# xyvirtualgroup/AdaptivePnP_SCI

Measured on NVIDIA B200. Metric: admm_iters_per_sec, higher is better.
Workload: dtype f16 operands / f32 accumulate (inference convs); tf32 / f32 (online update); f32 elsewhere

## Files before the change

adaptivepnp_sci_b200/csrc/sci_conv_tc.cu:

```cuda
#include <cuda.h>
#include <cuda_fp16.h>
#include <stdlib.h>

#include "sci_common.cuh"

int sci_conv3x3_ref_launch(const sci_conv_desc* d, void* stream);
int sci_wgrad_ref_launch(const sci_wgrad_desc* d, void* stream);

namespace {

constexpr int TILE_W = 16, TILE_H = 8;
constexpr int KCH = 32;
constexpr int A_BYTES = TILE_W * TILE_H * KCH * 4;
constexpr int TC_THREADS = 256;
constexpr int MAX_STAGES = 8;

struct FwdParams {
    const float* scale; const float* shift; const float* residual; float* y;
    int N, H, W, Ho, Wo, Cin, Cout, stride, relu, ps, round_tf32, wsplit, emit_lo;
    int tiles_w, tiles_h, num_tiles, k_chunks, stages, acc_stride, tmem_cols;
    int Cstore;
    int ks_last;
    int rb_in, a_bytes;
    int lo_chunk0;
// ... 282 lines not shown
                        for (int j = 0; j < 32; j += 8) {
                            uint32_t h[4];
#pragma unroll
                            for (int e = 0; e < 4; ++e) {
                                float t0 = v[j + 2 * e] * s_scale[c0 + j + 2 * e] + s_shift[c0 + j + 2 * e];
                                float t1 = v[j + 2 * e + 1] * s_scale[c0 + j + 2 * e + 1] + s_shift[c0 + j + 2 * e + 1];
                                if (p.relu) { t0 = fmaxf(t0, 0.f); t1 = fmaxf(t1, 0.f); }
                                h[e] = pack_half2(t0, t1);
                            }
                            if (j < nc) *reinterpret_cast<uint4*>(yp + j) = make_uint4(h[0], h[1], h[2], h[3]);
                        }
                    }
                } else if (valid) {
                    long o;
                    if (p.ps) {
                        const int qq = c0 / Cq, cc = c0 % Cq;
                        o = (((long)n * 2 * p.Ho + 2 * ho + (qq >> 1)) * 2 * p.Wo + 2 * wo + (qq & 1)) * Cq + cc;
                    } else {
                        o = (((long)n * p.Ho + ho) * p.Wo + wo) * (p.Cout << p.emit_lo) + c0;
                    }
#pragma unroll
                    for (int j = 0; j < 32; j += 4) {
                        if (j >= nc) break;
                        float4 r4 = make_float4(0.f, 0.f, 0.f, 0.f);
                        if (p.residual) r4 = *reinterpret_cast<const float4*>(p.residual + o + j);
                        float out[4], lo[4];
                        const float rr[4] = {r4.x, r4.y, r4.z, r4.w};
#pragma unroll
                        for (int e = 0; e < 4; ++e) {
                            float t = v[j + e] * s_scale[c0 + j + e] + s_shift[c0 + j + e];
                            if (p.relu) t = fmaxf(t, 0.f);
                            t += rr[e];
                            const float hi = p.round_tf32 ? rna_tf32(t) : t;
                            lo[e] = rna_tf32(t - hi);
                            out[e] = hi;
                        }
                        *reinterpret_cast<float4*>(p.y + o + j) = make_float4(out[0], out[1], out[2], out[3]);
                        if (p.emit_lo)
                            *reinterpret_cast<float4*>(p.y + o + p.Cout + j) = make_float4(lo[0], lo[1], lo[2], lo[3]);
                    }
                }
            }
            tc_fence_before();
            __syncwarp();
            if (lane == 0) mbar_arrive(&tempty_bar[acc]);
            if (++acc == 2) { acc = 0; acc_phase ^= 1u; }
        }
        if (lane == 0) asm volatile("cp.async.bulk.wait_group 0;" ::: "memory");
    }
    tc_fence_before();
    __syncthreads();
    if (warp == 2) {
        tc_fence_after();
        asm volatile("tcgen05.dealloc.cta_group::1.sync.aligned.b32 %0, %1;" ::"r"(tmem_base), "r"((uint32_t)p.tmem_cols) : "memory");
    }
}


constexpr int ROW_PX = 130;
constexpr int ROW_BYTES = ROW_PX * KCH * 4;
constexpr int A2_STAGE = 17 * 1024;

struct Fwd2Params {
    const float* scale; const float* shift; const float* residual; float* y;
    int N, H, W, Cin, Cout, relu, ps, round_tf32;
    int tiles_w, num_tiles, k_chunks, stages, acc_stride, tmem_cols, resident, out_bufs;
    const float* planar_in1; float* planar_out;
    int pdl;
    int col0, Ctot;
    int stack;
    int R, tiles_h;
    int dbg;
    int ucols, Cstore;
    const float* mask_y; float* col_s1; float* col_s2; int mask_relu;
    int split;
    int ks_last;
    int rb_in, rb_out, a_stage, row_bytes;
    uint32_t desc_hi;
};

template <int EPI_WG, int MODE, bool HALF>
__global__ void __launch_bounds__(128 + 128 * EPI_WG, 1)
conv_fwd2_tc_kernel(const __grid_constant__ CUtensorMap tmA, const __grid_constant__ CUtensorMap tmB,
                    const __grid_constant__ CUtensorMap tmY, const Fwd2Params p) {
    extern __shared__ uint8_t smem_raw[];
    __shared__ __align__(8) uint64_t full_bar[MAX_STAGES], empty_bar[MAX_STAGES], tfull_bar[2], tempty_bar[2], w_bar;
    __shared__ uint32_t tmem_slot;
    __shared__ __align__(16) float s_scale[128], s_shift[128];
    __shared__ float s_cs1[MODE == 4 ? 128 : 1], s_cs2[MODE == 4 ? 128 : 1];

    const int warp = threadIdx.x >> 5, lane = threadIdx.x & 31;
    if (MODE == 4) {
        for (int i = threadIdx.x; i < 128; i += 128 + 128 * EPI_WG) { s_cs1[i] = 0.f; s_cs2[i] = 0.f; }
    }
    const uint32_t smem_base = (smem_u32(smem_raw) + 1023u) & ~1023u;
    const uint32_t b_bytes = (uint32_t)p.Cout * (uint32_t)p.rb_in;
    const uint32_t w_bytes = p.resident ? 9u * (uint32_t)p.k_chunks * b_bytes : 0u;
    const bool wpair = !p.resident && p.R == 2;
    const uint32_t stage_bytes = (uint32_t)p.a_stage * (wpair ? 2u : 1u) + (p.resident ? 0u : 3u * b_bytes);
    const uint32_t ring_base = smem_base + w_bytes;
    const uint32_t stage_out_base = ring_base + (uint32_t)p.stages * stage_bytes;

    for (int i = threadIdx.x; i < p.Cout; i += 128 + 128 * EPI_WG) {
        s_scale[i] = p.scale ? p.scale[p.col0 + i] : 1.f;
        s_shift[i] = p.shift ? p.shift[p.col0 + i] : 0.f;
    }
    if (warp == 0 && lane == 0) {
        asm volatile("prefetch.tensormap [%0];" ::"l"(&tmA) : "memory");
        asm volatile("prefetch.tensormap [%0];" ::"l"(&tmB) : "memory");
    }
    if (warp == 1 && lane == 0) {
        for (int s = 0; s < p.stages; ++s) { mbar_init(&full_bar[s], 1); mbar_init(&empty_bar[s], 1); }
        for (int a = 0; a < 2; ++a) { mbar_init(&tfull_bar[a], 1); mbar_init(&tempty_bar[a], 4 * EPI_WG); }
        mbar_init(&w_bar, 1);
        asm volatile("fence.mbarrier_init.release.cluster;" ::: "memory");
        asm volatile("fence.proxy.async.shared::cta;" ::: "memory");
    }
    if (warp == 2) {
        asm volatile("tcgen05.alloc.cta_group::1.sync.aligned.shared::cta.b32 [%0], %1;" ::"r"(smem_u32(&tmem_slot)), "r"((uint32_t)p.tmem_cols) : "memory");
        asm volatile("tcgen05.relinquish_alloc_permit.cta_group::1.sync.aligned;" ::: "memory");
    }
    tc_fence_before();
    __syncthreads();
    tc_fence_after();
    const uint32_t tmem_base = __shfl_sync(0xffffffffu, tmem_slot, 0);
    asm volatile("griddepcontrol.launch_dependents;" ::: "memory");

    if (warp == 0) {
        if (p.resident) {
            if (elect_one()) {
                mbar_arrive_expect_tx(&w_bar, w_bytes);
                for (int tap = 0; tap < 9; ++tap)
                    for (int kc = 0; kc < p.k_chunks; ++kc) {
                        const uint32_t slot = p.stack ? (uint32_t)(((tap % 3) * p.k_chunks + kc) * 3 + tap / 3)
                                                      : (uint32_t)(tap * p.k_chunks + kc);
                        tma_load_3d(smem_base + slot * b_bytes, &tmB, &w_bar, kc * (HALF ? (p.rb_in >> 1) : KCH), p.col0, tap);
                    }
            }
            __syncwarp();
        }
        if (p.pdl) asm volatile("griddepcontrol.wait;" ::: "memory");
        int stage = 0; uint32_t phase = 0;
        for (int tile = blockIdx.x; tile < p.num_tiles; tile += gridDim.x) {
            const int wt = tile % p.tiles_w, hg = (tile / p.tiles_w) % p.tiles_h, n = tile / (p.tiles_w * p.tiles_h);
            const int y0 = hg * p.R, rows = min(p.R, p.H - y0);
            if (wpair) {
                for (int r = 0; r < 3; ++r) {
                    for (int kc = 0; kc < p.k_chunks; ++kc) {
                        mbar_wait(&empty_bar[stage], phase ^ 1u);
                        if (elect_one()) {
                            mbar_arrive_expect_tx(&full_bar[stage], 2u * (uint32_t)p.row_bytes + 3u * b_bytes);
                            const uint32_t a_dst = ring_base + (uint32_t)stage * stage_bytes;
                            const int cc = kc * (HALF ? (p.rb_in >> 1) : KCH);
                            tma_load_4d(a_dst, &tmA, &full_bar[stage], cc, wt * 128 - 1, y0 + r - 1, n);
                            tma_load_4d(a_dst + (uint32_t)p.a_stage, &tmA, &full_bar[stage], cc, wt * 128 - 1, y0 + r, n);
                            for (int s = 0; s < 3; ++s)
                                tma_load_3d(a_dst + 2u * (uint32_t)p.a_stage + (uint32_t)s * b_bytes, &tmB, &full_bar[stage], cc, p.col0, r * 3 + s);
                        }
                        __syncwarp();
                        if (++stage == p.stages) { stage = 0; phase ^= 1u; }
                    }
                }
                continue;
            }
            for (int j = 0; j < rows + 2; ++j) {
                for (int kc = 0; kc < p.k_chunks; ++kc) {
                    mbar_wait(&empty_bar[stage], phase ^ 1u);
                    if (elect_one()) {
                        const bool skip_a = (p.dbg & 2) != 0;
                        mbar_arrive_expect_tx(&full_bar[stage], (skip_a ? 0u : (uint32_t)p.row_bytes) + (p.resident ? 0u : 3u * b_bytes));
                        const uint32_t a_dst = ring_base + (uint32_t)stage * stage_bytes;
                        if (!skip_a) tma_load_4d(a_dst, &tmA, &full_bar[stage], kc * (HALF ? (p.rb_in >> 1) : KCH), wt * 128 - 1, y0 + j - 1, n);
                        if (!p.resident) {
                            for (int s = 0; s < 3; ++s)
                                tma_load_3d(a_dst + (uint32_t)p.a_stage + (uint32_t)s * b_bytes, &tmB, &full_bar[stage], kc * (HALF ? (p.rb_in >> 1) : KCH), p.col0, j * 3 + s);
                        }
                    }
                    __syncwarp();
                    if (++stage == p.stages) { stage = 0; phase ^= 1u; }
                }
            }
        }
    } else if (warp == 1) {
        const bool leader = elect_one();
        const uint32_t idesc = mma_idesc(HALF, p.Cout);
        if (p.resident) { mbar_wait(&w_bar, 0); tc_fence_after(); }
        int stage = 0; uint32_t phase = 0; int acc = 0; uint32_t acc_phase = 0;
        const uint32_t b_tile_lo = b_bytes >> 4;
        const uint32_t tapu = (uint32_t)p.rb_in >> 4;
        const int ks_full = p.rb_in >> 5;
        for (int tile = blockIdx.x; tile < p.num_tiles; tile += gridDim.x) {
            mbar_wait(&tempty_bar[acc], acc_phase ^ 1u);
            tc_fence_after();
            const int hg = (tile / p.tiles_w) % p.tiles_h;
            const int rows = min(p.R, p.H - hg * p.R);
            const uint32_t d_base = tmem_base + (uint32_t)(acc * p.R * p.acc_stride);
            if (p.R == 1) {
// ... 70 lines not shown
                    const int nr = r_hi - r_lo + 1;
                    const uint32_t d_col = d_base + (uint32_t)((p.R - 1 - (j - r_lo)) * p.acc_stride);
                    const uint32_t idesc_n = (idesc & ~(0x3Fu << 17)) | ((uint32_t)((nr * p.Cout) >> 3) << 17);
                    const uint32_t idesc_m = (idesc & ~(0x3Fu << 17)) | ((uint32_t)(((nr - 1) * p.Cout) >> 3) << 17);
                    for (int kc = 0; kc < p.k_chunks; ++kc) {
                        mbar_wait(&full_bar[stage], phase);
                        tc_fence_after();
                        if (leader) {
                            const uint32_t a_lo = desc_lo(ring_base + (uint32_t)stage * stage_bytes);
                            const int ksn = (kc == p.k_chunks - 1) ? p.ks_last : ks_full;
                            const uint32_t b_lo = desc_lo(smem_base + (uint32_t)(kc * 3 + r_lo) * b_bytes);
                            const uint32_t b_step = (uint32_t)(3 * p.k_chunks) * b_tile_lo;
                            if (p.dbg & 1) {
                            } else if (r_lo == 0 && kc == 0) {
                                mma_lo<HALF>(d_col, a_lo, b_lo, idesc, 0u, p.desc_hi);
                                if (nr > 1) mma_lo<HALF>(d_col + (uint32_t)p.acc_stride, a_lo, b_lo + b_tile_lo, idesc_m, 1u, p.desc_hi);
#pragma unroll
                                for (int sk = 1; sk < 3 * (KCH / 8); ++sk) {
                                    const int s = sk / (KCH / 8), k = sk % (KCH / 8);
                                    if (k < ksn) mma_lo<HALF>(d_col, a_lo + s * tapu + k * 2, b_lo + s * b_step + k * 2, idesc_n, 1u, p.desc_hi);
                                }
                            } else {
#pragma unroll
                                for (int s = 0; s < 3; ++s) {
#pragma unroll
                                    for (int k = 0; k < KCH / 8; ++k)
                                        if (k < ksn) mma_lo<HALF>(d_col, a_lo + s * tapu + k * 2, b_lo + s * b_step + k * 2, idesc_n, 1u, p.desc_hi);
                                }
                            }
                            tc_commit(&empty_bar[stage]);
                        }
                        __syncwarp();
                        if (++stage == p.stages) { stage = 0; phase ^= 1u; }
                    }
                }
            } else {
                for (int j = 0; j < rows + 2; ++j) {
                    for (int kc = 0; kc < p.k_chunks; ++kc) {
                        mbar_wait(&full_bar[stage], phase);
                        tc_fence_after();
                        if (leader) {
                            const uint32_t a_addr = ring_base + (uint32_t)stage * stage_bytes;
                            const uint32_t a_lo = desc_lo(a_addr);
                            const int ksn = (kc == p.k_chunks - 1) ? p.ks_last : ks_full;
                            for (int t = max(0, j - 2); t <= min(rows - 1, j); ++t) {
                                const int r = j - t;
                                const uint32_t d_tmem = d_base + (uint32_t)(t * p.acc_stride);
                                const uint32_t b_lo = desc_lo(p.resident ? smem_base + (uint32_t)(r * 3 * p.k_chunks + kc) * b_bytes : a_addr + (uint32_t)p.a_stage);
                                const uint32_t b_step = p.resident ? (uint32_t)p.k_chunks * b_tile_lo : b_tile_lo;
                                const uint32_t first = (uint32_t)((r | kc) != 0);
                                if (!(p.dbg & 1)) {
#pragma unroll
                                    for (int s = 0; s < 3; ++s) {
#pragma unroll
                                        for (int k = 0; k < KCH / 8; ++k)
                                            if (k < ksn) mma_lo<HALF>(d_tmem, a_lo + s * tapu + k * 2, b_lo + s * b_step + k * 2, idesc, (s | k) ? 1u : first, p.desc_hi);
                                    }
                                }
                            }
                            tc_commit(&empty_bar[stage]);
                        }
                        __syncwarp();
                        if (++stage == p.stages) { stage = 0; phase ^= 1u; }
                    }
                }
            }
            if (leader) tc_commit(&tfull_bar[acc]);
            __syncwarp();
            if (++acc == 2) { acc = 0; acc_phase ^= 1u; }
        }
    } else if (warp >= 4) {
        const int q = warp & 3;
        const int g = (warp >> 2) - 1;
        const int m = q * 32 + lane;
        const int Cq = p.Ctot >> 2;
        const int nch = p.Cout >> 5;
        const float lower = p.relu ? 0.f : -INFINITY;
        const long pl_plane = (long)p.H * p.W;
        constexpr int PIN_ROWS = (8 + EPI_WG - 1) / EPI_WG;
        const uint32_t tile_b = (uint32_t)p.rb_out * 32u;
        const uint32_t sbuf0 = stage_out_base + (uint32_t)((g * 4 + q) * p.out_bufs) * tile_b;
        int acc = 0; uint32_t acc_phase = 0;
        uint32_t st_cnt = 0;
        if (p.pdl) asm volatile("griddepcontrol.wait;" ::: "memory");
        for (int tile = blockIdx.x; tile < p.num_tiles; tile += gridDim.x) {
            const int wt = tile % p.tiles_w, hg = (tile / p.tiles_w) % p.tiles_h, n = tile / (p.tiles_w * p.tiles_h);
            const int y0 = hg * p.R, rows = min(p.R, p.H - y0);
            const int wo = wt * 128 + m;
            const bool valid = wo < p.W;
            const int units = rows * nch;
            auto out_offset = [&](int ho, int c0) -> long {
                const int cg = p.col0 + c0;
                if (p.ps) {
                    const int qq = cg / Cq, cc = cg % Cq;
                    return (((long)n * 2 * p.H + 2 * ho + (qq >> 1)) * 2 * p.W + 2 * wo + (qq & 1)) * Cq + cc;
                }
                return (((long)n * p.H + ho) * p.W + wo) * p.Ctot + cg;
            };
            float4 rr[8];
            float pin[PIN_ROWS][3];
            if (!HALF && MODE == 1) {
#pragma unroll
                for (int j = 0; j < 8; ++j) rr[j] = make_float4(0.f, 0.f, 0.f, 0.f);
                if (p.residual && valid && g < units) {
                    const float4* rp = reinterpret_cast<const float4*>(p.residual + out_offset(y0 + g / nch, (g % nch) << 5));
#pragma unroll
                    for (int j = 0; j < 8; ++j) rr[j] = __ldg(rp + j);
                }
            }
            if (MODE == 2) {
#pragma unroll
                for (int i = 0; i < PIN_ROWS; ++i) {
                    const int t = g + i * EPI_WG;
#pragma unroll
                    for (int c = 0; c < 3; ++c) pin[i][c] = 0.f;
                    if (valid && t < rows) {
                        const long o = (long)n * 3 * pl_plane + (long)(y0 + t) * p.W + wo;
#pragma unroll
                        for (int c = 0; c < 3; ++c) pin[i][c] = __ldg(p.planar_in1 + o + c * pl_plane);
                    }
                }
            }
            mbar_wait(&tfull_bar[acc], acc_phase);
            tc_fence_after();
            if (HALF && MODE != 2) {
                const int nun = (p.Cout + p.ucols - 1) / p.ucols;
                const int hunits = rows * nun;
                auto load_res = [&](int u, uint4 (&r)[8]) {
#pragma unroll
                    for (int j = 0; j < 8; ++j) r[j] = make_uint4(0u, 0u, 0u, 0u);
                    if (u < hunits && valid) {
                        const int t = u / nun, col0 = (u - t * nun) * p.ucols;
                        const int ncv = min(p.ucols, p.Cout - col0);
                        const int cg = p.col0 + col0, ho = y0 + t;
                        int qq = 0, cx = cg;
                        if (p.ps) { qq = cg / Cq; cx = cg - qq * Cq; }
                        const long pix = p.ps ? (((long)n * 2 * p.H + 2 * ho + (qq >> 1)) * 2 * p.W + 2 * wo + (qq & 1))
                                              : (((long)n * p.H + ho) * p.W + wo);
                        const uint4* rp = reinterpret_cast<const uint4*>(reinterpret_cast<const __half*>(p.residual) + pix * p.Cstore + cx);
#pragma unroll
                        for (int j = 0; j < 8; ++j)
                            if (j * 8 < ncv) r[j] = __ldg(rp + j);
                    }
                };
                uint4 rres[8];
                if (MODE == 1) load_res(g, rres);
                for (int u = g; u < hunits; u += EPI_WG) {
                    const int t = u / nun, col0 = (u - t * nun) * p.ucols;
                    const int ncv = min(p.ucols, p.Cout - col0);
                    const int ho = y0 + t;
                    const int cg = p.col0 + col0;
                    int qq = 0, cx = cg;
                    if (p.ps) { qq = cg / Cq; cx = cg - qq * Cq; }
                    uint4 rnext[8];
                    if (MODE == 1) load_res(u + EPI_WG, rnext);
                    const uint32_t t_row = tmem_base + (uint32_t)((acc * p.R + (p.stack ? p.R - 1 - t : t)) * p.acc_stride) + ((uint32_t)(q * 32) << 16);
                    uint32_t hv[32];
                    if (p.split) {
                        float v[32], sm[32];
                        tmem_ld32(t_row + col0, v);
                        tmem_ld32(t_row + p.Cout + col0, sm);
#pragma unroll
                        for (int j = 0; j < 32; j += 2) {
                            const float a0 = fmaxf(fmaf(fmaf(sm[j], 1.f / 2048.f, v[j]), s_scale[col0 + j], s_shift[col0 + j]), lower);
                            const float a1 = fmaxf(fmaf(fmaf(sm[j + 1], 1.f / 2048.f, v[j + 1]), s_scale[col0 + j + 1], s_shift[col0 + j + 1]), lower);
                            const uint32_t h = pack_half2(a0, a1);
                            const float2 hf = unpack_half2(h);
                            hv[j >> 1] = h;
                            hv[16 + (j >> 1)] = pack_half2((a0 - hf.x) * 2048.f, (a1 - hf.y) * 2048.f);
                        }
                        cx = 2 * cg;
                    } else
#pragma unroll
                    for (int hb = 0; hb < 2; ++hb) {
                        if (hb * 32 < ncv) {
                            float v[32];
                            tmem_ld32(t_row + col0 + hb * 32, v);
#pragma unroll
                            for (int j = 0; j < 32; j += 4) {
                                const float4 sc = *reinterpret_cast<const float4*>(&s_scale[col0 + hb * 32 + j]);
                                const float4 sh = *reinterpret_cast<const float4*>(&s_shift[col0 + hb * 32 + j]);
                                float a0 = fmaxf(fmaf(v[j], sc.x, sh.x), lower), a1 = fmaxf(fmaf(v[j + 1], sc.y, sh.y), lower);
                                float a2 = fmaxf(fmaf(v[j + 2], sc.z, sh.z), lower), a3 = fmaxf(fmaf(v[j + 3], sc.w, sh.w), lower);
                                if (MODE == 1) {
                                    const uint4 r4 = rres[hb * 4 + (j >> 3)];
                                    const float2 r0 = unpack_half2((j & 4) ? r4.z : r4.x), r1 = unpack_half2((j & 4) ? r4.w : r4.y);
                                    a0 += r0.x; a1 += r0.y; a2 += r1.x; a3 += r1.y;
                                }
                                hv[hb * 16 + (j >> 1)] = pack_half2(a0, a1);
                                hv[hb * 16 + (j >> 1) + 1] = pack_half2(a2, a3);
                            }
                        } else {
#pragma unroll
                            for (int j = 0; j < 16; ++j) hv[hb * 16 + j] = 0u;
                        }
                    }
                    const uint32_t sbuf = sbuf0 + (p.out_bufs == 2 ? (st_cnt & 1) * tile_b : 0u);
                    if (lane == 0) {
                        if (p.out_bufs == 2) asm volatile("cp.async.bulk.wait_group.read 1;" ::: "memory");
                        else                 asm volatile("cp.async.bulk.wait_group.read 0;" ::: "memory");
                    }
                    __syncwarp();
                    if (p.rb_out == 64) {
#pragma unroll
                        for (int j = 0; j < 4; ++j) {
                            const uint32_t a = sbuf + (uint32_t)lane * 64u + (uint32_t)((j ^ ((lane >> 1) & 3)) << 4);
                            asm volatile("st.shared.v4.b32 [%0], {%1, %2, %3, %4};" ::"r"(a), "r"(hv[4 * j]), "r"(hv[4 * j + 1]), "r"(hv[4 * j + 2]), "r"(hv[4 * j + 3]) : "memory");
                        }
                    } else {
#pragma unroll
                        for (int j = 0; j < 8; ++j) {
                            const uint32_t a = sbuf + (uint32_t)lane * 128u + (uint32_t)((j ^ (lane & 7)) << 4);
                            asm volatile("st.shared.v4.b32 [%0], {%1, %2, %3, %4};" ::"r"(a), "r"(hv[4 * j]), "r"(hv[4 * j + 1]), "r"(hv[4 * j + 2]), "r"(hv[4 * j + 3]) : "memory");
                        }
                    }
                    asm volatile("fence.proxy.async.shared::cta;" ::: "memory");
                    __syncwarp();
                    if (lane == 0) {
                        int cw = wt * 128 + q * 32, chh = ho;
                        if (p.ps) { cw = 2 * cw + (qq & 1); chh = 2 * ho + (qq >> 1); }
                        asm volatile("cp.async.bulk.tensor.4d.global.shared::cta.bulk_group [%0, {%2, %3, %4, %5}], [%1];"
                                     ::"l"(&tmY), "r"(sbuf), "r"(cx), "r"(cw), "r"(chh), "r"(n) : "memory");
                        asm volatile("cp.async.bulk.commit_group;" ::: "memory");
                    }
                    ++st_cnt;
                    if (MODE == 1) {
#pragma unroll
                        for (int j = 0; j < 8; ++j) rres[j] = rnext[j];
                    }
                }
            } else {
            auto unit = [&](int t, int c0, float (&v)[32]) {
                const uint32_t t_row = tmem_base + (uint32_t)((acc * p.R + (p.stack ? p.R - 1 - t : t)) * p.acc_stride) + ((uint32_t)(q * 32) << 16);
                tmem_ld32(t_row + c0, v);
#pragma unroll
                for (int j = 0; j < 32; j += 4) {
                    const float4 sc = *reinterpret_cast<const float4*>(&s_scale[c0 + j]);
                    const float4 sh = *reinterpret_cast<const float4*>(&s_shift[c0 + j]);
                    v[j]     = fmaxf(fmaf(v[j],     sc.x, sh.x), lower);
                    v[j + 1] = fmaxf(fmaf(v[j + 1], sc.y, sh.y), lower);
                    v[j + 2] = fmaxf(fmaf(v[j + 2], sc.z, sh.z), lower);
                    v[j + 3] = fmaxf(fmaf(v[j + 3], sc.w, sh.w), lower);
                }
            };
            if (MODE == 2) {
#pragma unroll
                for (int i = 0; i < PIN_ROWS; ++i) {
                    const int t = g + i * EPI_WG;
                    if (t < rows) {
                        float v[32];
                        unit(t, 0, v);
                        if (valid) {
                            const long o = (long)n * 3 * pl_plane + (long)(y0 + t) * p.W + wo;
#pragma unroll
                            for (int c = 0; c < 3; ++c) p.planar_out[o + c * pl_plane] = pin[i][c] - v[c];
                        }
                    }
                }
            } else {
                for (int u = g; u < units; u += EPI_WG) {
                    const int t = u / nch, c0 = (u - t * nch) << 5;
                    const int ho = y0 + t;
                    float v[32];
                    if (MODE == 4) {
                        float4 yy[8], ra[8];
                        const long eo = out_offset(ho, c0);
#pragma unroll
                        for (int j = 0; j < 8; ++j) { yy[j] = make_float4(0.f, 0.f, 0.f, 0.f); ra[j] = yy[j]; }
                        if (valid) {
                            const float4* yp = reinterpret_cast<const float4*>(p.mask_y + eo);
#pragma unroll
                            for (int j = 0; j < 8; ++j) yy[j] = __ldg(yp + j);
                            if (p.residual) {
                                const float4* rp = reinterpret_cast<const float4*>(p.residual + eo);
#pragma unroll
                                for (int j = 0; j < 8; ++j) ra[j] = __ldg(rp + j);
                            }
                        }
                        unit(t, c0, v);
                        const uint32_t sbuf = sbuf0;
                        if (lane == 0) asm volatile("cp.async.bulk.wait_group.read 0;" ::: "memory");
                        __syncwarp();
#pragma unroll
                        for (int j = 0; j < 8; ++j) {
                            const float ya[4] = {yy[j].x, yy[j].y, yy[j].z, yy[j].w};
                            const float rv[4] = {ra[j].x, ra[j].y, ra[j].z, ra[j].w};
                            float pz[4];
#pragma unroll
                            for (int e = 0; e < 4; ++e) {
                                float d = v[4 * j + e] + rv[e];
                                if (p.round_tf32) d = rna_tf32(d);
                                if (!valid || (p.mask_relu && !(ya[e] > 0.f))) d = 0.f;
                                v[4 * j + e] = d;
                                pz[e] = d * ya[e];
                            }
                            const uint32_t a = sbuf + (uint32_t)lane * 128u + (uint32_t)((j ^ (lane & 7)) << 4);
                            asm volatile("st.shared.v4.f32 [%0], {%1, %2, %3, %4};" ::"r"(a), "f"(pz[0]), "f"(pz[1]), "f"(pz[2]), "f"(pz[3]) : "memory");
                        }
                        __syncwarp();
                        float cs2 = 0.f;
                        if (p.col_s2) {
#pragma unroll 8
                            for (int r = 0; r < 32; ++r) {
                                float e;
                                const uint32_t a = sbuf + (uint32_t)r * 128u + (uint32_t)((((lane >> 2) ^ (r & 7)) << 4) + ((lane & 3) << 2));
                                asm volatile("ld.shared.f32 %0, [%1];" : "=f"(e) : "r"(a) : "memory");
                                cs2 += e;
                            }
                        }
                        __syncwarp();
#pragma unroll
                        for (int j = 0; j < 32; j += 4) {
// ... 231 lines not shown
    rc = make_weight_map(&tmB, d->w, d->Cout, d->Cin, 9 * (1 + p.wsplit), 0, half, rb_in == 64);
    if (rc) return rc;
    const size_t smem = (size_t)p.stages * stage_bytes + 1024;
    const int grid = min(p.num_tiles, SCI_NUM_SMS);
    p.pdl = (d->pdl && env_int("SCI_CONV_PDL", 1)) ? 1 : 0;
    if (env_int("SCI_CONV_VERBOSE", 0))
        fprintf(stderr, "conv v1 plan: %dx%d Cin %d -> %d stride %d half %d ps %d | tps %d stages %d lo_chunk0 %d ks_last %d wsplit %d "
                "emit_lo %d pdl %d tiles %d\n", d->H, d->W, d->Cin, d->Cout, d->stride, (int)half, p.ps, p.tps, p.stages, p.lo_chunk0,
                p.ks_last, p.wsplit, p.emit_lo, p.pdl, p.num_tiles);
    return launch(half ? conv_fwd_tc_kernel<true> : conv_fwd_tc_kernel<false>, dim3(grid), TC_THREADS, smem, stream, p.pdl,
                  "conv tc fwd", tmA, tmB, p);
}




bool fwd2_eligible(const sci_conv_desc* d) {
    if (d->planar_out) return true;
    if (d->half_io) return d->stride == 1;
    return d->stride == 1 && d->Cout % 32 == 0 && (d->Cout <= 128 || d->Cout == 256) && !d->w_split && !d->emit_lo &&
           env_int("SCI_CONV_V2", 1) != 0;
}

int conv_fwd2_tc_launch(const sci_conv_desc* d, void* stream, int col0, int ncols) {
    const bool half = d->half_io != 0;
    const int esz = half ? 2 : 4;
    const int rb_in = operand_row_bytes(d);
    const int kch = rb_in / esz;
    if (d->Cin % kch != 0) return sci_fail(SCI_EUNSUPPORTED, "conv tc v2: Cin % 32 (fp32) / % 64 or == 32 (fp16)");
    if (((uintptr_t)d->x | (uintptr_t)d->w | (uintptr_t)d->y | (uintptr_t)d->residual) & 15)
        return sci_fail(SCI_EINVAL, "conv tc: pointers must be 16-byte aligned");
    const int cin_store = (half && d->Cin_store) ? d->Cin_store : d->Cin;
    const int cout_store = (half && d->Cout_store) ? d->Cout_store : (d->pixel_shuffle ? d->Cout / 4 : d->Cout);
    if (half && (cin_store % 8 || cout_store % 8 || cin_store > d->Cin))
        return sci_fail(SCI_EINVAL, "conv tc v2 fp16: stored channel counts must be multiples of 8 (16-byte TMA strides)");
    Fwd2Params p;
    p.scale = d->scale; p.shift = d->shift; p.residual = d->residual; p.y = d->y;
    p.N = d->N; p.H = d->H; p.W = d->W; p.Cin = d->Cin; p.Cout = ncols; p.col0 = col0; p.Ctot = d->Cout;
    p.relu = d->relu; p.ps = d->pixel_shuffle; p.round_tf32 = d->round_tf32;
    p.planar_in1 = d->planar_in1; p.planar_out = d->planar_out;
    if (p.planar_out && (!p.planar_in1 || p.ps || p.Cout != 32 || d->residual))
        return sci_fail(SCI_EINVAL, "conv tc v2: planar output needs planar_in1, Cout == 32, no pixel_shuffle / residual");
    p.tiles_w = (p.W + 127) / 128;
    p.k_chunks = p.Cin / kch;
    const int rb_out = (half && cout_store == 32 && !p.planar_out) ? 64 : 128;
    p.rb_in = rb_in; p.rb_out = rb_out;
    p.a_stage = rb_in == 64 ? 9 * 1024 : A2_STAGE;
    p.row_bytes = ROW_PX * rb_in;
    p.desc_hi = rb_in == 64 ? DESC_HI_K64 : DESC_HI_K128;
    const int a_stage = p.a_stage;
    const int b_bytes = p.Cout * rb_in;
    const bool tma_store = !p.planar_out;
    p.Cstore = cout_store;
    p.ks_last = ks_last(d->Cin, (d->K_used > 0 && d->K_used <= d->Cin) ? d->K_used : d->Cin, rb_in, esz);
    p.ucols = 32;
    if (half) {
        const int cq = p.ps ? d->Cout / 4 : ncols;
        if (cq % 32 != 0) return sci_fail(SCI_EUNSUPPORTED, "conv tc v2 fp16: column groups of 32");
        p.ucols = (cq % 64 == 0 || cq > 64) ? 64 : 32;
        if (rb_out == 64 && p.ucols != 32) return sci_fail(SCI_EUNSUPPORTED, "conv tc v2 fp16: a 32-channel output tensor needs 32-column units");
        if (p.ps && cq != 32 && cq % 64 != 0) return sci_fail(SCI_EUNSUPPORTED, "conv tc v2 fp16: PixelShuffle groups of 32 or k*64 columns");
    }
    p.split = 0;
    if (half && d->w_split) {
        if (rb_in != 128 || p.ps || d->residual || p.planar_out || ncols != d->Cout || d->Cout % 32 || d->Cout > 128 || cout_store != 2 * d->Cout)
            return sci_fail(SCI_EUNSUPPORTED, "conv tc v2 fp16 split: plain layers, Cout % 32 == 0, Cout <= 128, Cout_store == 2 * Cout");
        p.split = (d->K_used > 0 && d->K_used <= 16 && p.k_chunks == 1) ? 1 : 2;
        p.ucols = 32;
        p.ks_last = 4;
    }
    int mode = p.planar_out ? 2 : (d->residual ? 1 : 0);
    p.mask_y = d->mask_y; p.col_s1 = d->col_s1; p.col_s2 = d->col_s2; p.mask_relu = d->mask_relu;
    if (d->mask_y) {
        if (half || p.planar_out || (d->pixel_shuffle ? d->Cout / 4 : d->Cout) > 128 || (d->col_s2 && !d->col_s1))
            return sci_fail(SCI_EUNSUPPORTED, "conv tc v2: fused activation backward needs the fp32 TMA-store path and <= 128 stored channels");
        mode = 4;
    }
    const int w_bytes = 9 * p.k_chunks * b_bytes;
    const int total_budget = 214 * 1024;
    const int tile_b = 32 * rb_out;
    int out_stage = 0, budget = 0, epi_wg = 2;
    const int epi_env = env_int("SCI_CONV_EPI_WG", 0);
    const int epi_first = epi_env ? (epi_env == 1 ? 1 : 2) : ((half || p.k_chunks <= 1 || d->residual || d->mask_y) ? 2 : 1);
    for (epi_wg = epi_first; epi_wg >= 1; --epi_wg) {
        for (p.out_bufs = ((epi_wg == 2 || d->mask_y) ? 1 : 2); p.out_bufs >= 1; --p.out_bufs) {
            out_stage = tma_store ? 4 * epi_wg * p.out_bufs * tile_b : 0;
            budget = total_budget - out_stage;
            p.resident = (w_bytes + 3 * a_stage <= budget) ? 1 : 0;
            const int sb = a_stage + (p.resident ? 0 : 3 * b_bytes);
            const int st = (budget - (p.resident ? w_bytes : 0)) / sb;
            const bool would_be_resident = w_bytes + 3 * a_stage <= total_budget - (tma_store ? 4 * epi_wg * tile_b : 0);
            if ((p.resident || !would_be_resident) && st >= 3) break;
            if (p.out_bufs == 1) break;
        }
        const bool resident_with_one = w_bytes + 3 * a_stage <= total_budget - (tma_store ? 4 * tile_b : 0);
        if (epi_wg == 1 || epi_env == 2 || half || p.resident || !resident_with_one) break;
    }
    if (env_int("SCI_CONV_RESIDENT", 1) == 0) p.resident = 0;
    int stage_bytes = a_stage + (p.resident ? 0 : 3 * b_bytes);
    p.stages = min(MAX_STAGES, (budget - (p.resident ? w_bytes : 0)) / stage_bytes);
    if (p.stages < 2) return sci_fail(SCI_EUNSUPPORTED, "conv tc v2: pipeline does not fit");
    p.acc_stride = p.split ? 2 * p.Cout : p.Cout;
    if (p.split && 2 * p.acc_stride > 512) return sci_fail(SCI_EUNSUPPORTED, "conv tc v2 fp16 split: accumulators do not fit");
    p.R = 1;
    if (!p.resident && !p.split && 2 * 2 * p.acc_stride <= 512 && p.H >= 2 && env_int("SCI_CONV_WPAIR", 1)) {
        const int sb2 = 2 * a_stage + 3 * b_bytes;
        const long tiles2 = (long)p.tiles_w * ((p.H + 1) / 2) * p.N;
        if (budget / sb2 >= 2 && tiles2 >= 8L * SCI_NUM_SMS) p.R = 2;
    }
    if (p.resident && !p.split) {
        const int rmax = env_int("SCI_CONV_ROWS", 8);
        while (p.R * 2 <= rmax && 2 * (p.R * 2) * p.acc_stride <= 512 && p.R * 2 <= p.H) p.R *= 2;
    }
    if (!p.resident && p.R == 2) {
        stage_bytes = 2 * a_stage + 3 * b_bytes;
        p.stages = min(MAX_STAGES, budget / stage_bytes);
    }
    p.stack = (p.resident && p.R >= 2 && 3 * p.Cout <= 256 && env_int("SCI_CONV_STACK", 1)) ? 1 : 0;
    p.tiles_h = (p.H + p.R - 1) / p.R;
    p.num_tiles = p.tiles_w * p.tiles_h * p.N;
    p.tmem_cols = next_pow2_cols(2 * p.R * p.acc_stride);
    p.dbg = env_int("SCI_CONV_DBG", 0);
    CUtensorMap tmA, tmB;
    int rc = make_act_map(&tmA, d->x, d->N, d->H, d->W, cin_store, 1, ROW_PX, 1,
                          rb_in == 64 ? CU_TENSOR_MAP_SWIZZLE_64B : CU_TENSOR_MAP_SWIZZLE_128B, half, rb_in == 64);
    if (rc) return rc;
    rc = make_weight_map(&tmB, d->w, d->Cout, d->Cin, 9, ncols, half, rb_in == 64);
    if (rc) return rc;
    CUtensorMap tmY = tmA;
    if (tma_store) {
        const int ps = d->pixel_shuffle ? 1 : 0;
        const cuuint64_t oc = (cuuint64_t)cout_store, ow = (cuuint64_t)(d->W << ps), oh = (cuuint64_t)(d->H << ps);
        const cuuint64_t dims[4] = {oc, ow, oh, (cuuint64_t)d->N};
        const cuuint64_t strides[3] = {oc * esz, ow * oc * esz, oh * ow * oc * esz};
        const cuuint32_t box[4] = {(cuuint32_t)(rb_out / esz), (cuuint32_t)(32 << ps), 1, 1};
        const cuuint32_t estr[4] = {1, (cuuint32_t)(1 << ps), 1, 1};
        rc = encode_map(&tmY, "output", d->y, half, 4, dims, strides, box, estr,
                        rb_out == 64 ? CU_TENSOR_MAP_SWIZZLE_64B : CU_TENSOR_MAP_SWIZZLE_128B, CU_TENSOR_MAP_L2_PROMOTION_NONE);
        if (rc) return rc;
    }
    const size_t smem = (size_t)(p.resident ? w_bytes : 0) + (size_t)p.stages * stage_bytes + out_stage + 1024;
    if (smem > 220 * 1024) return sci_fail(SCI_EUNSUPPORTED, "conv tc v2: shared memory budget exceeded");
    typedef void (*Fwd2Kernel)(const CUtensorMap, const CUtensorMap, const CUtensorMap, const Fwd2Params);
    static const Fwd2Kernel kernels[2][2][5] = {
        {{conv_fwd2_tc_kernel<1, 0, false>, conv_fwd2_tc_kernel<1, 1, false>, conv_fwd2_tc_kernel<1, 2, false>, nullptr,
          conv_fwd2_tc_kernel<1, 4, false>},
         {conv_fwd2_tc_kernel<2, 0, false>, conv_fwd2_tc_kernel<2, 1, false>, conv_fwd2_tc_kernel<2, 2, false>, nullptr,
          conv_fwd2_tc_kernel<2, 4, false>}},
        {{conv_fwd2_tc_kernel<1, 0, true>, conv_fwd2_tc_kernel<1, 1, true>, conv_fwd2_tc_kernel<1, 2, true>, nullptr, nullptr},
         {conv_fwd2_tc_kernel<2, 0, true>, conv_fwd2_tc_kernel<2, 1, true>, conv_fwd2_tc_kernel<2, 2, true>, nullptr, nullptr}}};
    const Fwd2Kernel kern = kernels[half ? 1 : 0][epi_wg - 1][mode];
    if (!kern) return sci_fail(SCI_EUNSUPPORTED, "conv tc v2: epilogue not built");
    const int grid = min(p.num_tiles, SCI_NUM_SMS);
    const int threads = 128 + 128 * epi_wg;
    p.pdl = (d->pdl && env_int("SCI_CONV_PDL", 1)) ? 1 : 0;
    if (env_int("SCI_CONV_VERBOSE", 0))
        fprintf(stderr, "conv v2 plan: %dx%d Cin %d -> %d cols (+%d) half %d ps %d mode %d | resident %d stages %d R %d stack %d epi_wg %d out_bufs %d "
                "rb %d/%d smem %zu KB tiles %d split %d ks_last %d pdl %d\n", d->H, d->W, d->Cin, ncols, col0, (int)half, p.ps, mode, p.resident,
                p.stages, p.R, p.stack, epi_wg, p.out_bufs, rb_in, rb_out, smem / 1024, p.num_tiles, p.split, p.ks_last, p.pdl);
    return launch(kern, dim3(grid), threads, smem, stream, p.pdl, "conv tc fwd v2", tmA, tmB, tmY, p);
}

constexpr int WG_TILE = 8;
constexpr int WG_CHUNK_BYTES = WG_TILE * WG_TILE * KCH * 4;

struct Wgrad2Params {
    const float* oscale; float* dw;
    int N, Ho, Wo, Cin, Cout, stride;
    int tiles_w, tiles_h, num_tiles;
    int swap, fuse, p_chunks, q_chunks, n_mma, accs, m_tiles, tmem_cols, stages;
};

__global__ void __launch_bounds__(TC_THREADS, 1)
conv_wgrad2_tc_kernel(const __grid_constant__ CUtensorMap tmZ, const __grid_constant__ CUtensorMap tmX, const Wgrad2Params p) {
    extern __shared__ uint8_t smem_raw[];
    __shared__ __align__(8) uint64_t full_bar[4], empty_bar[4], done_bar;
    __shared__ uint32_t tmem_slot;

    const int warp = threadIdx.x >> 5, lane = threadIdx.x & 31;
    const uint32_t smem_base = (smem_u32(smem_raw) + 1023u) & ~1023u;
    const int frow = blockIdx.y / p.m_tiles, mt = blockIdx.y % p.m_tiles;
    const int cin_chunks = p.Cin / KCH, cout_chunks = p.Cout / KCH;
    const int p_chunks = p.swap ? p.p_chunks : min(cout_chunks - mt * 4, 4);
    const uint32_t p_region = 4 * WG_CHUNK_BYTES;
    const uint32_t stage_bytes = p_region + (uint32_t)p.q_chunks * WG_CHUNK_BYTES;
    const uint32_t tx_bytes = (uint32_t)(p_chunks + p.q_chunks) * WG_CHUNK_BYTES;
    const int sub_steps = p.fuse ? 1 : 3;

    if (warp == 0 && lane == 0) {
        asm volatile("prefetch.tensormap [%0];" ::"l"(&tmZ) : "memory");
        asm volatile("prefetch.tensormap [%0];" ::"l"(&tmX) : "memory");
    }
    if (warp == 1 && lane == 0) {
        for (int s = 0; s < p.stages; ++s) { mbar_init(&full_bar[s], 1); mbar_init(&empty_bar[s], 1); }
        mbar_init(&done_bar, 1);
        asm volatile("fence.mbarrier_init.release.cluster;" ::: "memory");
        asm volatile("fence.proxy.async.shared::cta;" ::: "memory");
    }
    if (warp == 2) {
        asm volatile("tcgen05.alloc.cta_group::1.sync.aligned.shared::cta.b32 [%0], %1;" ::"r"(smem_u32(&tmem_slot)), "r"((uint32_t)p.tmem_cols) : "memory");
        asm volatile("tcgen05.relinquish_alloc_permit.cta_group::1.sync.aligned;" ::: "memory");
    }
    tc_fence_before();
    __syncthreads();
    tc_fence_after();
    const uint32_t tmem_base = __shfl_sync(0xffffffffu, tmem_slot, 0);

    if (warp == 0) {
        int stage = 0; uint32_t phase = 0;
        for (int tile = blockIdx.x; tile < p.num_tiles; tile += gridDim.x) {
            const int tw = tile % p.tiles_w, th = (tile / p.tiles_w) % p.tiles_h, n = tile / (p.tiles_w * p.tiles_h);
            const int ow0 = tw * WG_TILE, oh0 = th * WG_TILE;
            const int ix0 = ow0 * p.stride - 1, iy = oh0 * p.stride + frow - 1;
            for (int ss = 0; ss < sub_steps; ++ss) {
                mbar_wait(&empty_bar[stage], phase ^ 1u);
                if (elect_one()) {
                    mbar_arrive_expect_tx(&full_bar[stage], tx_bytes);
                    const uint32_t pb = smem_base + (uint32_t)stage * stage_bytes, qb = pb + p_region;
                    const uint32_t zb = p.swap ? qb : pb;
                    const int zc0 = p.swap ? 0 : mt * 4, zn = p.swap ? cout_chunks : p_chunks;
                    for (int c = 0; c < zn; ++c)
                        tma_load_4d(zb + c * WG_CHUNK_BYTES, &tmZ, &full_bar[stage], (zc0 + c) * KCH, ow0, oh0, n);
                    const uint32_t xb = p.swap ? pb : qb;
                    for (int s = (p.fuse ? 0 : ss); s < (p.fuse ? 3 : ss + 1); ++s)
                        for (int c = 0; c < cin_chunks; ++c)
                            tma_load_4d(xb + (uint32_t)((p.fuse ? s * cin_chunks : 0) + c) * WG_CHUNK_BYTES, &tmX, &full_bar[stage],
                                        c * KCH, ix0 + s, iy, n);
                }
                __syncwarp();
                if (++stage == p.stages) { stage = 0; phase ^= 1u; }
            }
        }
    } else if (warp == 1) {
        const uint32_t idesc = (1u << 4) | (2u << 7) | (2u << 10) | (1u << 15) | (1u << 16) |
                               ((uint32_t)(p.n_mma >> 3) << 17) | ((128u >> 4) << 24);
        const uint64_t desc_hi = umma_desc(0, WG_CHUNK_BYTES, 512, 1);
        int stage = 0; uint32_t phase = 0; uint32_t first = 1;
        for (int tile = blockIdx.x; tile < p.num_tiles; tile += gridDim.x) {
            for (int ss = 0; ss < sub_steps; ++ss) {
                mbar_wait(&full_bar[stage], phase);
                tc_fence_after();
                const uint32_t pb = smem_base + (uint32_t)stage * stage_bytes, qb = pb + p_region;
                const uint32_t d_tmem = tmem_base + (uint32_t)(ss * p.n_mma);
// ... 309 lines not shown
```

Measured before the change: 202.0.

## Load fp16 residual via TMA into output staging buffers instead of per-thread global loads

For the half-precision residual-add epilogue, the residual tile is now fetched with a 4D TMA bulk load into the existing double-buffered output staging smem, guarded by new per-warp mbarriers. Each warp prefetches the next unit's residual while processing the current one, then reads the residual back from swizzled shared memory. This replaces register-prefetched __ldg uint4 loads, aiming to cut register pressure and uncoalesced global traffic. It forces two output buffers in that mode, which can shrink the pipeline stage budget, and it adds waits on bulk store reads before each residual load.

```diff
diff --git a/adaptivepnp_sci_b200/csrc/sci_conv_tc.cu b/adaptivepnp_sci_b200/csrc/sci_conv_tc.cu
--- a/adaptivepnp_sci_b200/csrc/sci_conv_tc.cu
+++ b/adaptivepnp_sci_b200/csrc/sci_conv_tc.cu
@@ -388,9 +388,11 @@
 template <int EPI_WG, int MODE, bool HALF>
 __global__ void __launch_bounds__(128 + 128 * EPI_WG, 1)
 conv_fwd2_tc_kernel(const __grid_constant__ CUtensorMap tmA, const __grid_constant__ CUtensorMap tmB,
-                    const __grid_constant__ CUtensorMap tmY, const Fwd2Params p) {
+                    const __grid_constant__ CUtensorMap tmY, const __grid_constant__ CUtensorMap tmR, const Fwd2Params p) {
+    constexpr bool RES_TMA = HALF && MODE == 1;
     extern __shared__ uint8_t smem_raw[];
     __shared__ __align__(8) uint64_t full_bar[MAX_STAGES], empty_bar[MAX_STAGES], tfull_bar[2], tempty_bar[2], w_bar;
+    __shared__ __align__(8) uint64_t res_bar[RES_TMA ? 8 * EPI_WG : 1];
     __shared__ uint32_t tmem_slot;
     __shared__ __align__(16) float s_scale[128], s_shift[128];
     __shared__ float s_cs1[MODE == 4 ? 128 : 1], s_cs2[MODE == 4 ? 128 : 1];
@@ -414,11 +416,14 @@
     if (warp == 0 && lane == 0) {
         asm volatile("prefetch.tensormap [%0];" ::"l"(&tmA) : "memory");
         asm volatile("prefetch.tensormap [%0];" ::"l"(&tmB) : "memory");
+        if (RES_TMA) asm volatile("prefetch.tensormap [%0];" ::"l"(&tmR) : "memory");
     }
     if (warp == 1 && lane == 0) {
         for (int s = 0; s < p.stages; ++s) { mbar_init(&full_bar[s], 1); mbar_init(&empty_bar[s], 1); }
         for (int a = 0; a < 2; ++a) { mbar_init(&tfull_bar[a], 1); mbar_init(&tempty_bar[a], 4 * EPI_WG); }
         mbar_init(&w_bar, 1);
+        if (RES_TMA)
+            for (int i = 0; i < 8 * EPI_WG; ++i) mbar_init(&res_bar[i], 1);
         asm volatile("fence.mbarrier_init.release.cluster;" ::: "memory");
         asm volatile("fence.proxy.async.shared::cta;" ::: "memory");
     }
@@ -655,6 +660,8 @@
         const uint32_t sbuf0 = stage_out_base + (uint32_t)((g * 4 + q) * p.out_bufs) * tile_b;
         int acc = 0; uint32_t acc_phase = 0;
         uint32_t st_cnt = 0;
+        uint64_t* rbar = &res_bar[RES_TMA ? (g * 4 + q) * 2 : 0];
+        uint32_t res_ph = 0;
         if (p.pdl) asm volatile("griddepcontrol.wait;" ::: "memory");
         for (int tile = blockIdx.x; tile < p.num_tiles; tile += gridDim.x) {
             const int wt = tile % p.tiles_w, hg = (tile / p.tiles_w) % p.tiles_h, n = tile / (p.tiles_w * p.tiles_h);
@@ -694,30 +701,20 @@
                     }
                 }
             }
+            const int nun = (p.Cout + p.ucols - 1) / p.ucols;
+            const int hunits = rows * nun;
+            auto res_issue = [&](int u, uint32_t b) {
+                const int t = u / nun, cg = p.col0 + (u - t * nun) * p.ucols;
+                int cx = cg, cw = wt * 128 + q * 32, chh = y0 + t;
+                if (p.ps) { const int qq = cg / Cq; cx = cg - qq * Cq; cw = 2 * cw + (qq & 1); chh = 2 * chh + (qq >> 1); }
+                asm volatile("cp.async.bulk.wait_group.read 0;" ::: "memory");
+                mbar_arrive_expect_tx(&rbar[b], tile_b);
+                tma_load_4d(sbuf0 + b * tile_b, &tmR, &rbar[b], cx, cw, chh, n);
+            };
+            if (RES_TMA && g < hunits && lane == 0) res_issue(g, st_cnt & 1u);
             mbar_wait(&tfull_bar[acc], acc_phase);
             tc_fence_after();
             if (HALF && MODE != 2) {
-                const int nun = (p.Cout + p.ucols - 1) / p.ucols;
-                const int hunits = rows * nun;
-                auto load_res = [&](int u, uint4 (&r)[8]) {
-#pragma unroll
-                    for (int j = 0; j < 8; ++j) r[j] = make_uint4(0u, 0u, 0u, 0u);
-                    if (u < hunits && valid) {
-                        const int t = u / nun, col0 = (u - t * nun) * p.ucols;
-                        const int ncv = min(p.ucols, p.Cout - col0);
-                        const int cg = p.col0 + col0, ho = y0 + t;
-                        int qq = 0, cx = cg;
-                        if (p.ps) { qq = cg / Cq; cx = cg - qq * Cq; }
-                        const long pix = p.ps ? (((long)n * 2 * p.H + 2 * ho + (qq >> 1)) * 2 * p.W + 2 * wo + (qq & 1))
-                                              : (((long)n * p.H + ho) * p.W + wo);
-                        const uint4* rp = reinterpret_cast<const uint4*>(reinterpret_cast<const __half*>(p.residual) + pix * p.Cstore + cx);
-#pragma unroll
-                        for (int j = 0; j < 8; ++j)
-                            if (j * 8 < ncv) r[j] = __ldg(rp + j);
-                    }
-                };
-                uint4 rres[8];
-                if (MODE == 1) load_res(g, rres);
                 for (int u = g; u < hunits; u += EPI_WG) {
                     const int t = u / nun, col0 = (u - t * nun) * p.ucols;
                     const int ncv = min(p.ucols, p.Cout - col0);
@@ -725,8 +722,24 @@
                     const int cg = p.col0 + col0;
                     int qq = 0, cx = cg;
                     if (p.ps) { qq = cg / Cq; cx = cg - qq * Cq; }
-                    uint4 rnext[8];
-                    if (MODE == 1) load_res(u + EPI_WG, rnext);
+                    const uint32_t sbuf = sbuf0 + (p.out_bufs == 2 ? (st_cnt & 1) * tile_b : 0u);
+                    if (RES_TMA && u + EPI_WG < hunits && lane == 0) res_issue(u + EPI_WG, (st_cnt + 1) & 1u);
+                    uint4 rres[8];
+                    if (RES_TMA) {
+                        const uint32_t b = st_cnt & 1u;
+                        mbar_wait(&rbar[b], (res_ph >> b) & 1u);
+                        res_ph ^= 1u << b;
+#pragma unroll
+                        for (int j = 0; j < 8; ++j) {
+                            rres[j] = make_uint4(0u, 0u, 0u, 0u);
+                            if (j * 8 < ncv && (p.rb_out == 128 || j < 4)) {
+                                const uint32_t a = p.rb_out == 64 ? sbuf + (uint32_t)lane * 64u + (uint32_t)((j ^ ((lane >> 1) & 3)) << 4)
+                                                                  : sbuf + (uint32_t)lane * 128u + (uint32_t)((j ^ (lane & 7)) << 4);
+                                asm volatile("ld.shared.v4.b32 {%0, %1, %2, %3}, [%4];"
+                                             : "=r"(rres[j].x), "=r"(rres[j].y), "=r"(rres[j].z), "=r"(rres[j].w) : "r"(a) : "memory");
+                            }
+                        }
+                    }
                     const uint32_t t_row = tmem_base + (uint32_t)((acc * p.R + (p.stack ? p.R - 1 - t : t)) * p.acc_stride) + ((uint32_t)(q * 32) << 16);
                     uint32_t hv[32];
                     if (p.split) {
@@ -768,7 +781,6 @@
                             for (int j = 0; j < 16; ++j) hv[hb * 16 + j] = 0u;
                         }
                     }
-                    const uint32_t sbuf = sbuf0 + (p.out_bufs == 2 ? (st_cnt & 1) * tile_b : 0u);
                     if (lane == 0) {
                         if (p.out_bufs == 2) asm volatile("cp.async.bulk.wait_group.read 1;" ::: "memory");
                         else                 asm volatile("cp.async.bulk.wait_group.read 0;" ::: "memory");
@@ -797,10 +809,6 @@
                         asm volatile("cp.async.bulk.commit_group;" ::: "memory");
                     }
                     ++st_cnt;
-                    if (MODE == 1) {
-#pragma unroll
-                        for (int j = 0; j < 8; ++j) rres[j] = rnext[j];
-                    }
                 }
             } else {
             auto unit = [&](int t, int c0, float (&v)[32]) {
@@ -1198,8 +1206,9 @@
     int out_stage = 0, budget = 0, epi_wg = 2;
     const int epi_env = env_int("SCI_CONV_EPI_WG", 0);
     const int epi_first = epi_env ? (epi_env == 1 ? 1 : 2) : ((half || p.k_chunks <= 1 || d->residual || d->mask_y) ? 2 : 1);
+    const int min_bufs = (half && mode == 1) ? 2 : 1;
     for (epi_wg = epi_first; epi_wg >= 1; --epi_wg) {
-        for (p.out_bufs = ((epi_wg == 2 || d->mask_y) ? 1 : 2); p.out_bufs >= 1; --p.out_bufs) {
+        for (p.out_bufs = ((epi_wg == 2 || d->mask_y) ? min_bufs : 2); p.out_bufs >= min_bufs; --p.out_bufs) {
             out_stage = tma_store ? 4 * epi_wg * p.out_bufs * tile_b : 0;
             budget = total_budget - out_stage;
             p.resident = (w_bytes + 3 * a_stage <= budget) ? 1 : 0;
@@ -1207,7 +1216,7 @@
             const int st = (budget - (p.resident ? w_bytes : 0)) / sb;
             const bool would_be_resident = w_bytes + 3 * a_stage <= total_budget - (tma_store ? 4 * epi_wg * tile_b : 0);
             if ((p.resident || !would_be_resident) && st >= 3) break;
-            if (p.out_bufs == 1) break;
+            if (p.out_bufs == min_bufs) break;
         }
         const bool resident_with_one = w_bytes + 3 * a_stage <= total_budget - (tma_store ? 4 * tile_b : 0);
         if (epi_wg == 1 || epi_env == 2 || half || p.resident || !resident_with_one) break;
@@ -1243,7 +1252,7 @@
     if (rc) return rc;
     rc = make_weight_map(&tmB, d->w, d->Cout, d->Cin, 9, ncols, half, rb_in == 64);
     if (rc) return rc;
-    CUtensorMap tmY = tmA;
+    CUtensorMap tmY = tmA, tmR = tmA;
     if (tma_store) {
         const int ps = d->pixel_shuffle ? 1 : 0;
         const cuuint64_t oc = (cuuint64_t)cout_store, ow = (cuuint64_t)(d->W << ps), oh = (cuuint64_t)(d->H << ps);
@@ -1254,10 +1263,15 @@
         rc = encode_map(&tmY, "output", d->y, half, 4, dims, strides, box, estr,
                         rb_out == 64 ? CU_TENSOR_MAP_SWIZZLE_64B : CU_TENSOR_MAP_SWIZZLE_128B, CU_TENSOR_MAP_L2_PROMOTION_NONE);
         if (rc) return rc;
+        if (half && mode == 1) {
+            rc = encode_map(&tmR, "residual", d->residual, half, 4, dims, strides, box, estr,
+                            rb_out == 64 ? CU_TENSOR_MAP_SWIZZLE_64B : CU_TENSOR_MAP_SWIZZLE_128B);
+            if (rc) return rc;
+        }
     }
     const size_t smem = (size_t)(p.resident ? w_bytes : 0) + (size_t)p.stages * stage_bytes + out_stage + 1024;
     if (smem > 220 * 1024) return sci_fail(SCI_EUNSUPPORTED, "conv tc v2: shared memory budget exceeded");
-    typedef void (*Fwd2Kernel)(const CUtensorMap, const CUtensorMap, const CUtensorMap, const Fwd2Params);
+    typedef void (*Fwd2Kernel)(const CUtensorMap, const CUtensorMap, const CUtensorMap, const CUtensorMap, const Fwd2Params);
     static const Fwd2Kernel kernels[2][2][5] = {
         {{conv_fwd2_tc_kernel<1, 0, false>, conv_fwd2_tc_kernel<1, 1, false>, conv_fwd2_tc_kernel<1, 2, false>, nullptr,
           conv_fwd2_tc_kernel<1, 4, false>},
@@ -1274,7 +1288,7 @@
         fprintf(stderr, "conv v2 plan: %dx%d Cin %d -> %d cols (+%d) half %d ps %d mode %d | resident %d stages %d R %d stack %d epi_wg %d out_bufs %d "
                 "rb %d/%d smem %zu KB tiles %d split %d ks_last %d pdl %d\n", d->H, d->W, d->Cin, ncols, col0, (int)half, p.ps, mode, p.resident,
                 p.stages, p.R, p.stack, epi_wg, p.out_bufs, rb_in, rb_out, smem / 1024, p.num_tiles, p.split, p.ks_last, p.pdl);
-    return launch(kern, dim3(grid), threads, smem, stream, p.pdl, "conv tc fwd v2", tmA, tmB, tmY, p);
+    return launch(kern, dim3(grid), threads, smem, stream, p.pdl, "conv tc fwd v2", tmA, tmB, tmY, tmR, p);
 }
 
 constexpr int WG_TILE = 8;
```

Measured after the change: 203.4 (median of 6 runs). Within noise of the previous version (+0.7%).
